# teenylasers/eggshell

Measured on AMD Instinct MI355X. Metric: constraint_solve_steps_per_sec, higher is better.
Workload: dtype f64

## Files before the change

### eggshell_amd/capi.py

```python
import ctypes as C
import ctypes as _ct
import os
import weakref

import numpy as np

_HERE = os.path.dirname(os.path.abspath(__file__))
LIB_PATH = os.path.join(_HERE, "libeggshell_amd.so")

OK, ERR_INVALID, ERR_NO_DEVICE, ERR_HIP, ERR_STALL, ERR_UNSUPPORTED, ERR_LCP_FAILED, ERR_INTERNAL = range(8)
JACOBI, GAUSS_SEIDEL, SOR = 0, 1, 2
F64, F32 = 0, 1
JOINT_BALL, CONTACT_BOX, JOINT_LOCK, JOINT_HINGE_AXIS = 0, 1, 2, 3
JOINT_SLIDER_AXIS = 5
SHAPE_BOX, SHAPE_SPHERE, SHAPE_CAPSULE = 0, 1, 2
MV_LOWER, MV_UPPER, MV_DIAG, MV_FULL = 1, 2, 4, 8
SCHED_QUAD, SCHED_ISO, SCHED_QUAD_PATCHES, SCHED_LANE_PATCHES, SCHED_ALL_GLOBAL, SCHED_STATIC, SCHED_LEAN = 1, 2, 4, 8, 16, 32, 64
SCHED_LINSYM = 128
SCHED_FUSED_ASSEMBLY = 256
SCHED_DEFERRED_SYSTEM = 512
SCHED_START = 1024
SCHED_FRICTION = 2048
SCHED_PAIR = 4096
SCHED_CHAIN = 8192
SCHED_SHARE = 16384
SCHED_FACE = 32768
SCHED_FACE_SPLIT = 65536
START_RHS, START_GIVEN, START_PREVIOUS = 0, 1, 2
STABILIZE_INIT, STABILIZE_POST = 0, 1

EXPORTS = [
    "egs_default_params", "egs_context_create", "egs_context_destroy", "egs_last_error",
    "egs_context_synchronize", "egs_timer_start", "egs_timer_stop", "egs_kernel_time",
    "egs_solve_blocks", "egs_problem_create", "egs_problem_create_batch", "egs_problem_destroy", "egs_problem_set_blocks",
    "egs_problem_solve", "egs_problem_get_lambda", "egs_problem_get_accumulators",
    "egs_problem_set_state", "egs_problem_set_mass", "egs_problem_set_constraints", "egs_problem_assemble",
    "egs_problem_step", "egs_problem_get_blocks", "egs_problem_get_velocity",
    "egs_problem_advance", "egs_problem_get_state",
    "egs_problem_get_stats", "egs_problem_get_schedule", "egs_problem_get_schedule_full", "egs_problem_get_schedule_forms", "egs_mixed_constraints_solve", "egs_debug_plan", "egs_debug_plan_slots",
    "egs_update_contacts", "egs_update_contacts_joints", "egs_world_create", "egs_world_destroy", "egs_world_set_bodies",
    "egs_world_set_joints", "egs_world_step", "egs_world_get_bodies", "egs_world_get_contacts",
    "egs_world_get_lambda", "egs_world_info", "egs_world_create_batch", "egs_world_batch_info",
    "egs_problem_matvec", "egs_problem_get_matvec", "egs_problem_get_wres", "egs_matvec_blocks",
    "egs_debug_matvec_plan", "egs_debug_choose_oversize_schedule", "egs_debug_plan_timetable", "egs_debug_plan_pairable", "egs_debug_plan_chained", "egs_debug_plan_share", "egs_debug_plan_faced", "egs_debug_plan_face_normals", "egs_debug_face_split", "egs_box_lcp_dantzig", "egs_box_lcp_murty",
    "egs_box_lcp_batch", "egs_box_lcp_schur", "egs_box_lcp_schur_batch", "egs_dense_condition", "egs_dense_iterate", "egs_dense_iterate_batch", "egs_debug_plan_patches", "egs_problem_debug_trace",
    "egs_mixed_constraints_solve_limits", "egs_mixed_constraints_solve_batch", "egs_problem_dense_system", "egs_problem_dense_condition", "egs_problem_step_dense",
    "egs_world_step_dense", "egs_world_dense_info", "egs_world_stabilize", "egs_world_stabilize_info",
    "egs_world_stabilize_direct", "egs_world_stabilize_rank", "egs_relax_blocks_direct",
    "egs_world_step_each", "egs_world_step_dense_each",
    "egs_problem_set_start", "egs_match_contacts", "egs_world_set_warm_start", "egs_world_get_start",
    "egs_problem_set_friction", "egs_world_set_friction",
    "egs_update_contacts_shapes", "egs_world_set_shapes",
    "egs_mixed_friction_solve_batch", "egs_problem_set_dense_friction", "egs_problem_dense_friction_info",
    "egs_world_set_dense_friction", "egs_world_dense_friction_info",
    "egs_problem_set_live_inertia", "egs_problem_get_mass", "egs_world_set_live_inertia", "egs_world_get_mass",
    "egs_problem_set_restitution", "egs_world_set_restitution",
    "egs_problem_set_motors", "egs_world_set_joints_kinds", "egs_world_set_joint_motors", "egs_world_get_blocks",
    "egs_problem_set_hinge_limits", "egs_world_set_joint_limits",
    "egs_problem_set_slider_limits", "egs_world_set_slider_limits",
# ... 225 lines not shown
        if self.h:
            for child in list(self._children):
                child.close()
            load().egs_context_destroy(self.h)
            self.h = C.c_void_p()

    def __del__(self):
        try:
            self.close()
        except Exception:
            pass

    def synchronize(self):
        self.check(load().egs_context_synchronize(self.h))

    def timer_start(self):
        self.check(load().egs_timer_start(self.h))

    def timer_stop(self):
        ms = C.c_float(0)
        self.check(load().egs_timer_stop(self.h, C.byref(ms)))
        return ms.value

    def kernel_time(self, reset=True):
        s = C.c_double(0); n = C.c_int64(0)
        self.check(load().egs_kernel_time(self.h, C.byref(s), C.byref(n), C.c_int(1 if reset else 0)))
        return s.value, n.value

    def solve_blocks(self, Minv, body0, body1, J0, J1, is_eq, lo, hi, rhs, prm, precision=F64):
        Minv, J0, J1, lo, hi, rhs = map(_f64, (Minv, J0, J1, lo, hi, rhs))
# ... 546 lines not shown
    return bool(out.value)


def debug_face_split(n_tiles, slots, depth, period, sweeps, force=None):
    h, s1 = (-1, 0) if force is None else force
    tiles, cut, n = C.c_int32(0), C.c_int32(0), C.c_int32(0)
    pieces = np.zeros((2 * max(int(n_tiles), 0) + 1, 4), dtype=np.int32)
    st = load().egs_debug_face_split(C.c_int32(n_tiles), C.c_int32(slots), C.c_int32(depth), C.c_int32(period),
                                     C.c_int32(sweeps), C.c_int32(h), C.c_int32(s1), C.byref(tiles), C.byref(cut),
                                     _p(pieces), C.byref(n))
    if st != OK:
        raise EgsError(st, "egs_debug_face_split failed")
    return tiles.value, cut.value, pieces[:n.value].copy()


def debug_plan_face_normals(n_bodies, body0, body1, data):
    body0, body1 = _i32(body0), _i32(body1)
    data = np.ascontiguousarray(data, dtype=np.float64).reshape(body0.shape[0], 7)
    out = C.c_int32(0)
    st = load().egs_debug_plan_face_normals(C.c_int32(n_bodies), C.c_int32(body0.shape[0]), _p(body0), _p(body1), _p(data),
                                            C.byref(out))
    if st != OK:
        raise EgsError(st, "egs_debug_plan_face_normals failed")
    return bool(out.value)


class World:

    def __init__(self, ctx, n_bodies, precision=F64, _handle=None):
        self.ctx, self.n = ctx, int(n_bodies)
# ... 231 lines not shown
```

### eggshell_amd/csrc/context.cpp

```cpp
#include "plan.h"
#include "runtime.h"

using namespace egs;

extern "C" {

void egs_default_params(egs_solve_params *p) {
  if (!p) return;
  p->method = EGS_GAUSS_SEIDEL;
  p->max_iters = 500;
  p->check_every = 1;
  p->reserved = 0;
  p->omega = 1.5;
  p->cfm = 0.0;
  p->tol = 1e-9;
}

egs_status egs_context_create(int device_index, egs_context **out) {
  if (!out) return EGS_ERR_INVALID;
  *out = nullptr;
  int count = 0;
  if (hipGetDeviceCount(&count) != hipSuccess || count <= 0) return EGS_ERR_NO_DEVICE;
  if (device_index < 0 || device_index >= count) return EGS_ERR_INVALID;
  egs_context *ctx = new (std::nothrow) egs_context;
// ... 30 lines not shown
  if (ctx->oneshot) { egs_problem_destroy(ctx->oneshot); ctx->oneshot = nullptr; }
  for (auto e : ctx->kev) if (e) (void)hipEventDestroy(e);
  if (ctx->t0) (void)hipEventDestroy(ctx->t0);
  if (ctx->t1) (void)hipEventDestroy(ctx->t1);
  if (ctx->stream) (void)hipStreamDestroy(ctx->stream);
  delete ctx;
}

const char *egs_last_error(const egs_context *ctx) { return ctx ? ctx->error.c_str() : "no context"; }

egs_status egs_context_synchronize(egs_context *ctx) {
  if (!ctx) return EGS_ERR_INVALID;
  return guarded(ctx, [&]() -> egs_status { HIPCHK(hipStreamSynchronize(ctx->stream)); return EGS_OK; });
}

egs_status egs_timer_start(egs_context *ctx) {
  if (!ctx) return EGS_ERR_INVALID;
  return guarded(ctx, [&]() -> egs_status { HIPCHK(hipEventRecord(ctx->t0, ctx->stream)); return EGS_OK; });
}

egs_status egs_timer_stop(egs_context *ctx, float *elapsed_ms) {
  if (!ctx || !elapsed_ms) return EGS_ERR_INVALID;
  return guarded(ctx, [&]() -> egs_status {
    HIPCHK(hipEventRecord(ctx->t1, ctx->stream));
    HIPCHK(hipEventSynchronize(ctx->t1));
    HIPCHK(hipEventElapsedTime(elapsed_ms, ctx->t0, ctx->t1));
    return EGS_OK;
  });
}

// ... 20 lines not shown
```

### eggshell_amd/csrc/kernels.h

```cpp
#pragma once
#include <hip/hip_runtime.h>

#include <cstdint>
#include <type_traits>

#include "plan.h"

namespace egs {

struct AssembleCore {
  int32_t n, m;
  const double *pos, *R, *v, *w;
  const double *Wf;
  const int32_t *kind, *body0, *body1;
  const double *data;
  double dt, erp;
  void *J0, *J1, *lo, *hi, *rhs;
  double *err;
  uint8_t *is_eq;
};
struct AssembleArgs : AssembleCore {
  const double *rest = nullptr;
  double vth = 0.0;
};
// ... 76 lines not shown
void launch_step_solve(const SolveArgs<REAL> &a, int method, int n_tiles, int block, int group, bool linsym, hipStream_t s);
void launch_step_solve_assemble(const SolveArgs<double> &a, int method, int n_tiles, bool store_system, hipStream_t s);
void launch_step_solve_pair(const SolveArgs<double> &a, int method, int n_tiles, bool store_system, bool chain, bool share,
                            hipStream_t s);
struct FacePiece;
struct FaceWork {
  const FacePiece *pieces;
  uint32_t *counter;
  uint32_t *flags;
  uint32_t ticket_base, epoch;
  int32_t n_pieces;
  int32_t n_workgroups;
  double *v6;
  int32_t *host_stall;
};
void launch_step_solve_face(const SolveArgs<double> &a, int n_tiles, int tiles_per_cu, const FaceWork &w, hipStream_t s);
template <typename REAL>
void launch_step_quad(const SolveArgs<REAL> &a, int method, int n_tiles, int tile_size, hipStream_t s);
template <typename REAL>
void launch_global_solve(const GlobalArgs<REAL> &a, int max_blocks, hipStream_t s);
template <typename REAL> int occupancy_global_solve();
template <typename REAL> int occupancy_patch_solve(size_t lds_bytes);
template <typename REAL> int occupancy_quad_patch_solve(size_t lds_bytes);
template <typename REAL> int occupancy_step_quad(int tile_size, size_t lds_bytes);
template <typename REAL>
void launch_global_wres(const GlobalArgs<REAL> &a, hipStream_t s);
template <typename REAL>
void launch_patch_solve(const SolveArgs<REAL> &a, int method, int n_tiles, uint32_t *tickets, hipStream_t s);
template <typename REAL>
void launch_cons_prepare(const SolveArgs<REAL> &a, hipStream_t s);
template <typename REAL>
// ... 70 lines not shown
```

### eggshell_amd/csrc/plan_debug.cpp

```cpp
#include <exception>

#include "../../include/eggshell_amd.h"
#include "matvec_plan.h"
#include "plan.h"
#include "policy.h"

using namespace egs;

namespace {

template <typename F>
egs_status plan_entry(int32_t n, int32_t m, const int32_t *body0, const int32_t *body1, F &&f) {
  if (n < 0 || m < 0 || (m > 0 && (!body0 || !body1))) return EGS_ERR_INVALID;
  try {
    return f();
  } catch (const std::exception &) {
    return EGS_ERR_INVALID;
  }
}

template <typename LANE, typename F>
void for_each_constraint_lane(const std::vector<LANE> &lanes, int n_tiles, int block, F &&f) {
  for (int t = 0; t < n_tiles; ++t)
    for (int l = 0; l < block; ++l) {
// ... 170 lines not shown
    if (s1) *s1 = f.s1;
    std::vector<FacePiece> list;
    face_piece_list(n_tiles, slots, f, sweeps, list);
    if (n_pieces) *n_pieces = (int32_t)list.size();
    if (pieces)
      for (size_t i = 0; i < list.size(); ++i) {
        pieces[4 * i] = list[i].tile; pieces[4 * i + 1] = list[i].resume;
        pieces[4 * i + 2] = list[i].sweeps; pieces[4 * i + 3] = list[i].kind;
      }
    return EGS_OK;
  } catch (const std::exception &) {
    return EGS_ERR_INVALID;
  }
}

}
```

### eggshell_amd/csrc/policy.h

```cpp
#pragma once

#include <algorithm>

#include "../../include/eggshell_amd.h"
#include "plan.h"

namespace egs {

inline int quad_tiles_per_cu_max(int precision) { return precision == EGS_F32 ? 8 : 5; }
constexpr int kBigTileMinConstraints = 196608;
inline bool timetable_pays(const Plan &pl, int sweeps) {
  const double grp = pl.runs ? 4.0 : 1.0;
  const double fixed = grp * ((double)pl.max_depth + (double)pl.max_period * sweeps);
  const double ticket = grp * (double)pl.max_depth + (double)pl.max_cnt * sweeps;
  return fixed <= 1.15 * ticket;
}

enum OversizeSchedule { kQuadPatches = 0, kLanePatches = 1, kAllGlobal = 2 };
inline OversizeSchedule choose_oversize_schedule(int n_patch_tiles, int quad_per_cu, int patch_per_cu, int cu_count,
                                                 bool patches_enabled, bool quad_patches_enabled) {
  if (n_patch_tiles <= 0 || !patches_enabled) return kAllGlobal;
  const long quad_cap = (long)std::min(quad_per_cu, 1) * cu_count, lane_cap = (long)std::min(patch_per_cu, 2) * cu_count;
  if (quad_patches_enabled && n_patch_tiles <= quad_cap) return kQuadPatches;
  if (n_patch_tiles <= lane_cap) return kLanePatches;
  return kAllGlobal;
}

constexpr int kFaceTilesPerCu = 4;

constexpr int kFaceSplitPrologueSteps = 260;
struct FaceSplit {
  int tiles = 0;
  int s1 = 0;
};
inline FaceSplit face_split_policy(long n_tiles, long slots, int depth, int P, int S) {
  FaceSplit f;
  if (slots <= 0 || n_tiles <= slots || S < 2 || P <= 0) return f;
  const long R = n_tiles % slots;
  if (R == 0 || 2 * R > slots) return f;
  const int s1 = S / 2;
  if ((long)P * (S - s1) <= (long)depth + kFaceSplitPrologueSteps) return f;
  f.tiles = (int)R;
  f.s1 = s1;
// ... 31 lines not shown
  for (long i = 0; i < total; ++i) {
    if (done_f < H && (done_w >= beside || done_f * total <= i * (long)H)) {
      out.push_back(FacePiece{whole + (int)done_f, 0, f.s1, kFaceFirst});
      ++done_f;
    } else {
      out.push_back(FacePiece{t++, 0, S, kFaceWhole});
      ++done_w;
    }
  }
  for (; t < whole; ++t) out.push_back(FacePiece{t, 0, S, kFaceWhole});
  for (int h = 0; h < H; ++h) out.push_back(FacePiece{whole + h, 1, S - f.s1, kFaceSecond});
}

inline bool face_persist_pays(long n_tiles, long slots) { return slots > 0 && n_tiles > slots; }

inline bool iso_schedule_pays(long m, int cu, int precision) {
  const long t = (m + 255) / 256;
  if (precision == EGS_F32) return t > 3L * cu;
  if (t < 2L * cu) return false;
  const long full3 = t / (3L * cu), rem3 = t % (3L * cu);
  const double iso = 0.50 * full3 + (rem3 == 0 ? 0.0 : rem3 <= cu ? 0.435 : rem3 <= 2L * cu ? 0.462 : 0.50);
  const double regular = 0.415 * ((t / 2 + cu - 1) / cu);
  return iso < regular;
}

}
```

### eggshell_amd/csrc/problem.h

```cpp
#pragma once

#include "kernels.h"
#include "matvec_plan.h"
#include "plan.h"
#include "policy.h"
#include "runtime.h"

namespace egs {

struct DevicePlan {
  DevBuf<LaneDesc> lanes;
  DevBuf<uint16_t> lane_level;
  DevBuf<int32_t> tile_period, tile_depth;
  DevBuf<int32_t> tile_nslots, tile_slot_off, slot_body;
  void stage(egs_context *ctx, const Plan &pl) {
    egs::stage(ctx, lanes, pl.lanes);
    egs::stage(ctx, lane_level, pl.lane_level);
    egs::stage(ctx, tile_period, pl.tile_period);
    egs::stage(ctx, tile_depth, pl.tile_depth);
    egs::stage(ctx, tile_nslots, pl.tile_nslots);
    egs::stage(ctx, tile_slot_off, pl.tile_slot_off);
    egs::stage(ctx, slot_body, pl.slot_body);
  }
};
// ... 10 lines not shown

}

struct egs_problem {
  egs_context *ctx = nullptr;
  int n = 0, m = 0, precision = EGS_F64;
  egs::Plan plan;
  bool tile_plan_ready = false;
  std::vector<int32_t> h_body0, h_body1;
  egs::DevicePlan tile;
  egs::Plan planq;
  bool use_quad = false;
  uint32_t last_sched = 0;
  static constexpr uint32_t kSchedRefinements = EGS_SCHED_CHAIN;
  static constexpr uint32_t kSchedFullOnly = EGS_SCHED_SHARE;
  static constexpr uint32_t kSchedFormsOnly = EGS_SCHED_FACE | EGS_SCHED_FACE_SPLIT;
  bool lin_neg = false;
  bool joint_pairs = false;
  bool contacts_only = false;
  int linsym_bodies = -1;
  static constexpr int kShareUndecided = -1, kShareDeviceData = -2;
  int share_normals = kShareDeviceData;
  bool face_normals = false;
  int oversize = 2;
  int global_max_blocks = 1;
  egs::DevicePlan quad;
  egs::DevBuf<unsigned char> wsB0, wsB1, wsD, wsInv;
  egs::DevBuf<egs::GlobalDesc> gcons;
  egs::DevBuf<uint32_t> gtickets;
  egs::DevBuf<unsigned long long> trace;
  int trace_sweeps = 0;
// ... 151 lines not shown
```

### eggshell_amd/csrc/solve.cpp

```cpp
#include <algorithm>
#include <cmath>
#include <cstdio>
#include <limits>

#include "policy.h"
#include "problem.h"
#include "stabilize.h"

namespace egs {
namespace {

struct SweepSchedule {
  bool quad = false;
  bool timetable = false;
  int iso = 0;
  int group = 1;
  bool linsym = false;
  bool assemble = false;
  bool defer = false;
  bool pair = false;
  bool chain = false;
  bool share = false;
  bool face = false;
  int face_tiles = kFaceTilesPerCu;
  FaceSplit split;
  long face_slots = 0;
  bool face_persistent = false;
  bool started = false;
  bool friction = false;
  int steady = 0;
  int oversize = -1;
  uint32_t flags() const {
    return (iso ? EGS_SCHED_ISO : 0) | (timetable ? EGS_SCHED_STATIC : 0) | (linsym ? EGS_SCHED_LINSYM : 0) |
           (assemble ? EGS_SCHED_FUSED_ASSEMBLY : 0) | (defer ? EGS_SCHED_DEFERRED_SYSTEM : 0) |
           (started ? EGS_SCHED_START : 0) | (friction ? EGS_SCHED_FRICTION : 0) | (pair ? EGS_SCHED_PAIR : 0) |
           (chain ? EGS_SCHED_CHAIN : 0) | (share ? EGS_SCHED_SHARE : 0) |
           (face ? EGS_SCHED_FACE : 0) | (split.tiles > 0 ? EGS_SCHED_FACE_SPLIT : 0);
  }
};

SweepSchedule choose_sweep(egs_problem *p, int method, int sweeps, bool hist, bool resume, bool offer_assembly) {
  SweepSchedule s;
  s.started = p->start_active;
  s.friction = p->friction;
  s.quad = p->use_quad && method != EGS_JACOBI;
  if (!s.quad) ensure_tile_plan(p);
  const Plan &pl = s.quad ? p->planq : p->plan;
  const char *se = std::getenv("EGS_STEP");
  s.timetable = method != EGS_JACOBI && pl.levels_ok && pl.n_tiles > 0 && (se ? std::atoi(se) != 0 : timetable_pays(pl, sweeps));
  if (s.quad) return s;
  const char *ye = std::getenv("EGS_STEP_STEADY");
  s.steady = s.timetable && !(ye && std::atoi(ye) == 0);
// ... 11 lines not shown
  s.linsym = !f32 && s.group == 1 && p->lin_neg && p->linsym_bodies == 1 && !(le && std::atoi(le) == 0);
  const char *fe = std::getenv("EGS_FUSED_ASSEMBLY");
  s.assemble = offer_assembly && s.linsym && p->contacts_only && !s.friction && !resume && !solve_takes_start(p) && pl.global.empty() && !(fe && std::atoi(fe) == 0);
  const char *de = std::getenv("EGS_STEP_DEFER_SYSTEM");
  s.defer = s.assemble && !(de && std::atoi(de) == 0);
  const char *pe = std::getenv("EGS_STEP_PAIR");
  s.pair = s.assemble && pl.pairable && !(pe && std::atoi(pe) == 0);
  const char *ce = std::getenv("EGS_STEP_CHAIN");
  s.chain = s.pair && pl.chained && s.steady && !(ce && std::atoi(ce) == 0);
  const char *he = std::getenv("EGS_STEP_SHARE");
  if (s.chain && p->share_normals == egs_problem::kShareUndecided) decide_share_normals(p);
  s.share = s.chain && p->share_normals == 1 && !(he && std::atoi(he) == 0);
  const char *ae = std::getenv("EGS_STEP_FACE"), *te = std::getenv("EGS_STEP_FACE_TILES");
  s.face = s.share && pl.faced && p->face_normals && method == EGS_GAUSS_SEIDEL && s.defer && !p->restitution &&
           !(ae && std::atoi(ae) == 0);
  if (te && (std::atoi(te) == 3 || std::atoi(te) == 4)) s.face_tiles = std::atoi(te);
  const char *xe = std::getenv("EGS_STEP_FACE_SPLIT"), *xf = std::getenv("EGS_STEP_FACE_SPLIT_FORCE");
  const char *ke = std::getenv("EGS_STEP_FACE_SLOTS");
  s.face_slots = ke && std::atol(ke) > 0 ? std::atol(ke) : (long)p->ctx->cu_count * s.face_tiles;
  if (s.face && !(xe && std::atoi(xe) == 0)) {
    long h = 0, s1 = 0;
    if (xf && std::sscanf(xf, "%ld,%ld", &h, &s1) == 2) s.split = face_split_forced(pl.n_tiles, h, s1, sweeps);
    else if (!xf) s.split = face_split_policy(pl.n_tiles, s.face_slots, pl.max_depth, pl.max_period, sweeps);
    const char *re = std::getenv("EGS_STEP_FACE_PERSIST");
    s.face_persistent = s.split.tiles > 0 || (face_persist_pays(pl.n_tiles, s.face_slots) && !(re && std::atoi(re) == 0));
  }
  return s;
}

template <typename ARGS, typename REAL>
void system_args(ARGS &a, const egs_problem *p, REAL cfm, bool hist) {
  a.m = p->m; a.n_bodies = p->n;
  a.Minv = real<REAL>(p->Minv_r);
// ... 69 lines not shown
  hipStream_t st = p->ctx->stream;
  if (!sc.assemble) {
    launch_step_solve<REAL>(a, method, n_tiles, p->plan.block, sc.group, sc.linsym, st);
    return;
  }
  if constexpr (sizeof(REAL) == 8) {
    a.assemble = *assemble;
    if (sc.face) {
      FaceWork w = sc.face_persistent ? face_work(p, n_tiles, sc.face_slots, sc.split, sweeps) : FaceWork{};
      w.host_stall = p->h_flag_dev;
      const char *ve = std::getenv("EGS_STEP_FACE_VELOCITY");
      if (p->step_velocity == egs_problem::kVelocityOffered && p->plan_covers_bodies && !(ve && std::atoi(ve) == 0)) {
        w.v6 = p->v6.p;
        p->step_velocity = egs_problem::kVelocityWritten;
      }
      launch_step_solve_face(a, n_tiles, sc.face_tiles, w, st);
    } else if (sc.pair) launch_step_solve_pair(a, method, n_tiles, !sc.defer, sc.chain, sc.share, st);
    else launch_step_solve_assemble(a, method, n_tiles, !sc.defer, st);
    p->sys_deferred = sc.defer;
    p->deferred_prev = false;
    p->deferred_dt = assemble->dt; p->deferred_erp = assemble->erp;
  }
}

template <typename REAL>
void launch_solve_t(egs_problem *p, int method, REAL cfm, REAL kscale, int sweeps, int resume, const AssembleArgs *assemble) {
  egs_context *ctx = p->ctx;
  const bool hist = p->hist_sweeps > 0;
  const SweepSchedule sc = choose_sweep(p, method, sweeps, hist, resume, assemble != nullptr);
  if (assemble && !sc.assemble)
    throw std::logic_error("fused assembly offered to a launch that does not take it");
// ... 495 lines not shown
```

### eggshell_amd/csrc/step_face.hip

```cpp
#include <algorithm>

#include "kernels.h"
#include "policy.h"
#include "step_device.h"
#include "step_pair_device.h"

namespace egs {

namespace {

#ifndef EGS_FACE_ANG_PRODUCTS
#define EGS_FACE_ANG_PRODUCTS 6
#endif
constexpr int kFaceLin = 9, kFaceAng = EGS_FACE_ANG_PRODUCTS;
constexpr int kFaceThreads = 128, kFaceLanes = 256;

struct FaceBodies {
  double pos0[3], pos1[3];
  double u0[6], u1[6];
  double wl0, wa0, wl1, wa1;
  bool has0, has1;
};
__device__ __forceinline__ void face_bodies(const SolveArgs<double> &A, int b0, int b1, FaceBodies &B) {
  const AssembleArgs &G = A.assemble;
  const size_t i0 = (size_t)max(b0, 0), i1 = (size_t)max(b1, 0);
  double vw0[6], vw1[6], wf0[6], wf1[6];
#pragma unroll
  for (int k = 0; k < 3; ++k) {
    B.pos0[k] = G.pos[i0 * 3 + k];
    B.pos1[k] = G.pos[i1 * 3 + k];
// ... 26 lines not shown
  double e[3];
  contact_blocks(d, B.pos0, B.pos1, has0, has1, c.J0, c.J1, e);
#pragma unroll
  for (int r = 0; r < 3; ++r) c.rhs[r] = assemble_rhs(A.assemble, c.J0, c.J1, e, B.u0, B.u1, r);
  c.wl0 = B.wl0; c.wa0 = B.wa0; c.wl1 = B.wl1; c.wa1 = B.wa1;
  load_cons<double, true, false, true, false, true>(A, 0, has0, has1, 0, 0, c);
#pragma unroll
  for (int r = 0; r < 3; ++r) {
    c.rhs[r] = active ? c.rhs[r] : 0.0;
    c.inv[r] = active ? c.inv[r] : 0.0;
    asm volatile("" : "+v"(c.rhs[r]), "+v"(c.inv[r]));
    x[r] = c.rhs[r];
  }
  asm volatile("" : "+v"(c.D[3]), "+v"(c.D[6]), "+v"(c.D[7]));
}
template <bool LIN>
__device__ __forceinline__ void face_sides(const Cons<double> &c, int side, PairLin<kFaceLin> &L, PairAng<kFaceAng> &GE,
                                           PairAng<kFaceAng> &GO) {
#pragma unroll
  for (int r = 0; r < 3; ++r) {
#pragma unroll
    for (int k = 0; k < 3; ++k) {
      const double ga = dpp_all<kQuadSwap>(side ? c.J0[6 * r + 3 + k] : c.J1[6 * r + 3 + k]);
      GE.J[3 * r + k] = side ? ga : c.J0[6 * r + 3 + k];
      GO.J[3 * r + k] = side ? c.J1[6 * r + 3 + k] : ga;
      if constexpr (LIN) {
        const double gl = dpp_all<kQuadSwap>(c.J1[6 * r + k]);
        L.J[3 * r + k] = side ? gl : c.J0[6 * r + k];
      }
    }
  }
  if constexpr (LIN) {
    const double gl = dpp_all<kQuadSwap>(c.wl1), ga = dpp_all<kQuadSwap>(c.wa1);
    L.wl = side ? gl : c.wl0;
    L.wa = side ? ga : c.wa0;
  }
}

template <bool PIECES>
__device__ __forceinline__ bool face_step(const SolveArgs<double> &A, const FaceWork &W, unsigned char *smem, const int tid) {
  constexpr int METHOD = 1;
  int tile = blockIdx.x, n_sweeps = A.sweeps, resume = 0, kind = kFaceWhole;
  if constexpr (PIECES) {
    unsigned *s_word = reinterpret_cast<unsigned *>(smem);
    if (tid == 0) *s_word = atomicAdd(W.counter, 1u) - W.ticket_base;
    __syncthreads();
    const unsigned ticket = (unsigned)__builtin_amdgcn_readfirstlane((int)*s_word);
    __syncthreads();
    if (ticket >= (unsigned)W.n_pieces) return false;
    const FacePiece pc = W.pieces[ticket];
    tile = __builtin_amdgcn_readfirstlane(pc.tile);
    resume = __builtin_amdgcn_readfirstlane(pc.resume);
    n_sweeps = __builtin_amdgcn_readfirstlane(pc.sweeps);
    kind = __builtin_amdgcn_readfirstlane(pc.kind);
  }
  const int side = tid & 1;
// ... 18 lines not shown

  const int own0 = side ? dm[1].cidx : dm[0].cidx, own1 = side ? dm[3].cidx : dm[2].cidx;
  double d0[7], d1[7];
#pragma unroll
  for (int k = 0; k < 7; ++k) {
    d0[k] = A.assemble.data[(size_t)max(own0, 0) * 7 + k];
    d1[k] = A.assemble.data[(size_t)max(own1, 0) * 7 + k];
  }
  const int body0 = slot_body[slot0], body1 = slot_body[slot1];
  __builtin_amdgcn_sched_barrier(0);
  FaceBodies B;
  B.has0 = slot0 != 0;
  B.has1 = slot1 != 0;
  face_bodies(A, body0, body1, B);

  PairLin<kFaceLin> L;
  PairAng<kFaceAng> GA, GB, GC, GD;
  Cons<double> c0 = {}, c1 = {};
  double x0[3], x1[3];
  face_assemble(A, d0, B, own0 >= 0, c0, x0);
  face_sides<true>(c0, side, L, GA, GB);
#pragma unroll
  for (int e = 0; e < 9; ++e) {
    s_acc[e * kFaceThreads + tid] = L.J[e];
    s_acc[(9 + e) * kFaceThreads + tid] = GA.J[e];
    s_acc[(18 + e) * kFaceThreads + tid] = GB.J[e];
  }
  asm volatile("" ::: "memory");
  __builtin_amdgcn_sched_barrier(0);
  face_assemble(A, d1, B, own1 >= 0, c1, x1);
  __builtin_amdgcn_sched_barrier(0);
  asm volatile("" ::: "memory");
#pragma unroll
  for (int e = 0; e < 9; ++e) {
    L.J[e] = s_acc[e * kFaceThreads + tid];
    GA.J[e] = s_acc[(9 + e) * kFaceThreads + tid];
    GB.J[e] = s_acc[(18 + e) * kFaceThreads + tid];
  }
  face_sides<false>(c1, side, L, GC, GD);
  __syncthreads();
  if (PIECES && resume) {
    unsigned *s_word = reinterpret_cast<unsigned *>(smem);
    if (tid == 0) {
      uint32_t spins = 0;
      unsigned ok = 1;
      while (__hip_atomic_load(W.flags + tile, __ATOMIC_ACQUIRE, __HIP_MEMORY_SCOPE_AGENT) != W.epoch) {
        if (++spins > A.spin_limit) { ok = 0; break; }
        __builtin_amdgcn_s_sleep(8);
      }
      *s_word = ok;
    }
    __syncthreads();
    const bool ok = __builtin_amdgcn_readfirstlane((int)*s_word) != 0;
    __builtin_amdgcn_fence(__ATOMIC_ACQUIRE, "agent");
    __syncthreads();
// ... 13 lines not shown
      const int body = slot_body[s];
#pragma unroll
      for (int k = 0; k < 6; ++k) s_acc[s * 6 + k] = body >= 0 ? A.acc[(size_t)body * 6 + k] : 0.0;
    }
  } else {
    for (int s = tid; s < nslots; s += kFaceThreads) {
#pragma unroll
      for (int k = 0; k < 6; ++k) s_acc[s * 6 + k] = 0.0;
    }
  }
  L.form();
  GA.form(L.wa);
  GB.form(L.wa);
  GC.form(L.wa);
  GD.form(L.wa);
  PairShared<kFaceLin, kFaceAng> SA{L, GA}, SB{L, GB}, SC{L, GC}, SD{L, GD};
  const int t_end = __builtin_amdgcn_readfirstlane(timetable_end<METHOD>(depth, P, n_sweeps, resume));
  __syncthreads();

  int sweep = resume, due = (nm > 0 && n_sweeps >= resume) ? levelA : 0x7fffffff;
  int t_s = 0, t_e = 0;
  const int Ps = __builtin_amdgcn_readfirstlane(P);
  if (A.steady && Ps > 0) {
    t_s = (__builtin_amdgcn_readfirstlane(depth) + 3) & ~3;
    t_e = min(Ps * (n_sweeps + 1 - resume), t_end);
    t_e -= (t_e - t_s) & 3;
    if (t_e <= t_s) t_s = t_e = 0;
  }
  int t = 0, stop = t_e > t_s ? t_s : t_end;
  double a[6];
  for (;;) {
    for (; t < stop; t += 4) {
      if (due == t) {
        pair_pass<METHOD, kQuadEven, true, true, false>(SA, ac, a, has, even, c0, x0, sweep, A.cfm);
        if (nm > 1) pair_pass<METHOD, kQuadOdd, true, false, false>(SB, ac, a, has, odd, c0, x0, sweep, A.cfm);
        if (nm > 2) pair_pass<METHOD, kQuadEven, true, false, false>(SC, ac, a, has, even, c1, x1, sweep, A.cfm);
        if (nm > 3) pair_pass<METHOD, kQuadOdd, true, false, false>(SD, ac, a, has, odd, c1, x1, sweep, A.cfm);
        if (has) store6(ac, a);
        due += P;
        if (++sweep > n_sweeps) due = 0x7fffffff;
      }
      asm volatile("s_waitcnt lgkmcnt(0)" ::: "memory");
      __builtin_amdgcn_s_barrier();
    }
    if (t >= t_end) break;
    {
      const int phF = nm > 0 ? levelA % Ps : -1;
      int tp = t % Ps;
      for (; t < t_e; t += 4) {
        if (phF == tp) {
          pair_pass<METHOD, kQuadEven, false, true, false>(SA, ac, a, has, even, c0, x0, 1, A.cfm);
          if (nm > 1) pair_pass<METHOD, kQuadOdd, false, false, false>(SB, ac, a, has, odd, c0, x0, 1, A.cfm);
          if (nm > 2) pair_pass<METHOD, kQuadEven, false, false, false>(SC, ac, a, has, even, c1, x1, 1, A.cfm);
          if (nm > 3) pair_pass<METHOD, kQuadOdd, false, false, false>(SD, ac, a, has, odd, c1, x1, 1, A.cfm);
          if (has) store6(ac, a);
        }
        asm volatile("s_waitcnt lgkmcnt(0)" ::: "memory");
        __builtin_amdgcn_s_barrier();
        tp = tp + 4 == Ps ? 0 : tp + 4;
      }
    }
    const int lv = A.lane_level[lane0];
    const int n = t_e > lv ? (t_e - lv + Ps - 1) / Ps : 0;
    sweep = n + resume;
    due = (nm == 0 || sweep > n_sweeps) ? 0x7fffffff : lv + P * n;
    stop = t_end;
  }

  const int cidx0 = A.lanes[lane0 + 32 * side].cidx, cidx1 = A.lanes[lane0 + 64 + 32 * side].cidx;
  if (nm > 0) pair_epilogue(A, SA, ac, even, cidx0, c0, x0);
  if (nm > 1) pair_epilogue(A, SB, ac, odd, cidx0, c0, x0);
  if (nm > 2) pair_epilogue(A, SC, ac, even, cidx1, c1, x1);
  if (nm > 3) pair_epilogue(A, SD, ac, odd, cidx1, c1, x1);
  for (int s = tid + 1; s < nslots; s += kFaceThreads) {
    const int body = slot_body[s];
    if (body < 0) continue;
    double acc[6];
#pragma unroll
    for (int k = 0; k < 6; ++k) A.acc[(size_t)body * 6 + k] = acc[k] = s_acc[s * 6 + k];
    if (W.v6 && kind != kFaceFirst) {
      const AssembleArgs &G = A.assemble;
#pragma unroll
      for (int k = 0; k < 6; ++k) {
        const double vel = k < 3 ? G.v[(size_t)body * 3 + k] : G.w[(size_t)body * 3 + k - 3];
        W.v6[(size_t)body * 6 + k] = vel + G.dt * (G.Wf[(size_t)body * 6 + k] + acc[k]);
      }
    }
  }
  if (PIECES && kind == kFaceFirst) {
    __builtin_amdgcn_fence(__ATOMIC_RELEASE, "agent");
    __syncthreads();
    if (tid == 0) __hip_atomic_store(W.flags + tile, W.epoch, __ATOMIC_RELEASE, __HIP_MEMORY_SCOPE_AGENT);
  }
  return true;
}

__global__ void __launch_bounds__(kFaceThreads, 2) step_solve_face_kernel(const SolveArgs<double> A, const FaceWork W) {
  extern __shared__ __attribute__((aligned(16))) unsigned char smem[];
  face_step<false>(A, W, smem, (int)threadIdx.x);
}
__global__ void __launch_bounds__(kFaceThreads, 2) step_solve_face_pieces_kernel(const SolveArgs<double> A, const FaceWork W) {
  extern __shared__ __attribute__((aligned(16))) unsigned char smem[];
  int tid = (int)threadIdx.x;
  for (;;) {
    SolveArgs<double> B = A;
    asm volatile("" : "+v"(tid), "+s"(B.assemble.dt), "+s"(B.assemble.erp), "+s"(B.cfm));
    if (!face_step<true>(B, W, smem, tid)) break;
    __syncthreads();
  }
}

}

void launch_step_solve_face(const SolveArgs<double> &a, int n_tiles, int tiles_per_cu, const FaceWork &w, hipStream_t s) {
  if (n_tiles <= 0) return;
  SolveArgs<double> b = a;
  b.n_tiles = n_tiles;
  size_t lds = std::max((size_t)b.max_slots * 6, (size_t)27 * kFaceThreads) * sizeof(double);
  constexpr size_t kQuarterLds = 160 * 1024 / 4;
  if (tiles_per_cu == 3) lds = std::max(lds, kQuarterLds + 1024);
  if (w.pieces) launch_lds(step_solve_face_pieces_kernel, dim3(w.n_workgroups), dim3(kFaceThreads), lds, s, b, w);
  else launch_lds(step_solve_face_kernel, dim3(n_tiles), dim3(kFaceThreads), lds, s, b, w);
}

}
```

### include/eggshell_amd.h

```cpp
#ifndef EGGSHELL_AMD_H
#define EGGSHELL_AMD_H

#include <stdint.h>

#ifdef __cplusplus
extern "C" {
#endif

typedef struct egs_context egs_context;
typedef struct egs_problem egs_problem;

typedef enum {
  EGS_OK = 0,
  EGS_ERR_INVALID = 1,
  EGS_ERR_NO_DEVICE = 2,
  EGS_ERR_HIP = 3,
  EGS_ERR_STALL = 4,
  EGS_ERR_UNSUPPORTED = 5,
  EGS_ERR_LCP_FAILED = 6,
  EGS_ERR_INTERNAL = 7
} egs_status;

typedef enum { EGS_JACOBI = 0, EGS_GAUSS_SEIDEL = 1, EGS_SOR = 2 } egs_method;
typedef enum { EGS_F64 = 0, EGS_F32 = 1 } egs_precision;
// ... 27 lines not shown
  EGS_SCHED_ISO = 2,
  EGS_SCHED_QUAD_PATCHES = 4,
  EGS_SCHED_LANE_PATCHES = 8,
  EGS_SCHED_ALL_GLOBAL = 16,
  EGS_SCHED_STATIC = 32,
  EGS_SCHED_LEAN = 64,
  EGS_SCHED_LINSYM = 128,
  EGS_SCHED_FUSED_ASSEMBLY = 256,
  EGS_SCHED_DEFERRED_SYSTEM = 512,
  EGS_SCHED_START = 1024,
  EGS_SCHED_FRICTION = 2048,
  EGS_SCHED_PAIR = 4096,
  EGS_SCHED_CHAIN = 8192,
  EGS_SCHED_SHARE = 16384,
  EGS_SCHED_FACE = 32768,
  EGS_SCHED_FACE_SPLIT = 65536
} egs_schedule_flags;

void egs_default_params(egs_solve_params *p);

egs_status egs_context_create(int device_index, egs_context **out);
void egs_context_destroy(egs_context *ctx);
const char *egs_last_error(const egs_context *ctx);
egs_status egs_context_synchronize(egs_context *ctx);
egs_status egs_timer_start(egs_context *ctx);
egs_status egs_timer_stop(egs_context *ctx, float *elapsed_ms);
egs_status egs_kernel_time(egs_context *ctx, double *sum_ms, int64_t *launches,
                           int reset);

egs_status egs_solve_blocks(egs_context *ctx, int32_t n_bodies,
                            const double *Minv, int32_t m,
                            const int32_t *body0, const int32_t *body1,
                            const double *J0, const double *J1,
                            const uint8_t *is_eq, const double *lo,
                            const double *hi, const double *rhs,
                            const egs_solve_params *params, int32_t precision,
                            double *x, egs_solve_stats *stats);

egs_status egs_problem_create(egs_context *ctx, int32_t n_bodies, int32_t m,
// ... 247 lines not shown
                                  int32_t *chained);

egs_status egs_debug_plan_share(int32_t n_bodies, int32_t m, const int32_t *body0, const int32_t *body1,
                                const double *data, int32_t *share);

egs_status egs_debug_plan_faced(int32_t n_bodies, int32_t m, const int32_t *body0, const int32_t *body1,
                                int32_t *faced);

egs_status egs_debug_plan_face_normals(int32_t n_bodies, int32_t m, const int32_t *body0, const int32_t *body1,
                                       const double *data, int32_t *face);

egs_status egs_debug_face_split(int32_t n_tiles, int32_t slots, int32_t depth, int32_t period, int32_t sweeps,
                                int32_t force_tiles, int32_t force_s1, int32_t *split_tiles, int32_t *s1,
                                int32_t *pieces, int32_t *n_pieces);

int32_t egs_debug_choose_oversize_schedule(int32_t n_patch_tiles, int32_t quad_per_cu,
                                           int32_t patch_per_cu, int32_t cu_count,
                                           int32_t patches_enabled, int32_t quad_patches_enabled);

egs_status egs_debug_matvec_plan(int32_t n_bodies, int32_t m, const int32_t *body0,
                                 const int32_t *body1, int32_t tile_size, int32_t *n_tiles,
                                 int32_t *n_islands, int32_t *n_shared_bodies,
                                 int32_t *n_boundary, int32_t *cons_tile, int32_t *cons_lane);

egs_status egs_cast_rays(egs_context *ctx, int32_t n_bodies, const double *pos, const double *R,
                         const double *side_lengths, const int32_t *shape ,
                         int32_t n_rays, const int32_t *ray_body ,
                         const double *origin, const double *dir, const double *tmax,
                         int32_t *hit_body, double *t, double *normal );
egs_status egs_world_set_rays(egs_world *w, int32_t n_rays, const int32_t *ray_ens ,
// ... 9 lines not shown
```

Before: 55770.

## Add lean FACE kernel variant with LDS-parked constraints for higher occupancy

Adds a lean form of the FACE step kernel that drops the angular product registers and parks per-constraint rhs, diagonal and inverse values in LDS, so it can run three workgroups per SIMD and six tiles per CU. A cost model (face_form_policy) picks lean or normal per problem by estimating launch time from piece count and block steps. The aim is higher occupancy and fewer persistent pieces on large problems. The price is extra LDS traffic on every pass and recomputed products, and lean is used only when the tile count exceeds the normal slot count and the model favours it.

```diff
diff --git a/eggshell_amd/capi.py b/eggshell_amd/capi.py
--- a/eggshell_amd/capi.py
+++ b/eggshell_amd/capi.py
@@ -26,12 +26,13 @@
 SCHED_SHARE = 16384
 SCHED_FACE = 32768
 SCHED_FACE_SPLIT = 65536
+SCHED_FACE_LEAN = 131072
 START_RHS, START_GIVEN, START_PREVIOUS = 0, 1, 2
 STABILIZE_INIT, STABILIZE_POST = 0, 1
 
 EXPORTS = [
     "egs_default_params", "egs_context_create", "egs_context_destroy", "egs_last_error",
-    "egs_context_synchronize", "egs_timer_start", "egs_timer_stop", "egs_kernel_time",
+    "egs_context_synchronize", "egs_context_cu_count", "egs_timer_start", "egs_timer_stop", "egs_kernel_time",
     "egs_solve_blocks", "egs_problem_create", "egs_problem_create_batch", "egs_problem_destroy", "egs_problem_set_blocks",
     "egs_problem_solve", "egs_problem_get_lambda", "egs_problem_get_accumulators",
     "egs_problem_set_state", "egs_problem_set_mass", "egs_problem_set_constraints", "egs_problem_assemble",
@@ -42,7 +43,7 @@
     "egs_world_set_joints", "egs_world_step", "egs_world_get_bodies", "egs_world_get_contacts",
     "egs_world_get_lambda", "egs_world_info", "egs_world_create_batch", "egs_world_batch_info",
     "egs_problem_matvec", "egs_problem_get_matvec", "egs_problem_get_wres", "egs_matvec_blocks",
-    "egs_debug_matvec_plan", "egs_debug_choose_oversize_schedule", "egs_debug_plan_timetable", "egs_debug_plan_pairable", "egs_debug_plan_chained", "egs_debug_plan_share", "egs_debug_plan_faced", "egs_debug_plan_face_normals", "egs_debug_face_split", "egs_box_lcp_dantzig", "egs_box_lcp_murty",
+    "egs_debug_matvec_plan", "egs_debug_choose_oversize_schedule", "egs_debug_plan_timetable", "egs_debug_plan_pairable", "egs_debug_plan_chained", "egs_debug_plan_share", "egs_debug_plan_faced", "egs_debug_plan_face_normals", "egs_debug_face_split", "egs_debug_face_form", "egs_box_lcp_dantzig", "egs_box_lcp_murty",
     "egs_box_lcp_batch", "egs_box_lcp_schur", "egs_box_lcp_schur_batch", "egs_dense_condition", "egs_dense_iterate", "egs_dense_iterate_batch", "egs_debug_plan_patches", "egs_problem_debug_trace",
     "egs_mixed_constraints_solve_limits", "egs_mixed_constraints_solve_batch", "egs_problem_dense_system", "egs_problem_dense_condition", "egs_problem_step_dense",
     "egs_world_step_dense", "egs_world_dense_info", "egs_world_stabilize", "egs_world_stabilize_info",
@@ -298,6 +299,11 @@
     def synchronize(self):
         self.check(load().egs_context_synchronize(self.h))
 
+    def cu_count(self):
+        n = C.c_int32(0)
+        self.check(load().egs_context_cu_count(self.h, C.byref(n)))
+        return n.value
+
     def timer_start(self):
         self.check(load().egs_timer_start(self.h))
 
@@ -874,6 +880,19 @@
     return tiles.value, cut.value, pieces[:n.value].copy()
 
 
+def debug_face_form(n_tiles, cus, depth, period, sweeps, max_slots=0):
+    lean, lds = C.c_int32(0), C.c_int64(0)
+    us, split = np.zeros(2, dtype=np.float64), np.zeros((2, 2), dtype=np.int32)
+    lib = load()
+    lib.egs_debug_face_form.argtypes = [C.c_int32] * 6 + [C.c_void_p] * 4
+    st = lib.egs_debug_face_form(n_tiles, cus, depth, period, sweeps, max_slots, C.addressof(lean), us.ctypes.data,
+                                 split.ctypes.data, C.addressof(lds))
+    if st != OK:
+        raise EgsError(st, "egs_debug_face_form failed")
+    return {"lean": bool(lean.value), "us": (float(us[0]), float(us[1])),
+            "split": (tuple(int(v) for v in split[0]), tuple(int(v) for v in split[1])), "lds_bytes": int(lds.value)}
+
+
 def debug_plan_face_normals(n_bodies, body0, body1, data):
     body0, body1 = _i32(body0), _i32(body1)
     data = np.ascontiguousarray(data, dtype=np.float64).reshape(body0.shape[0], 7)
diff --git a/eggshell_amd/csrc/context.cpp b/eggshell_amd/csrc/context.cpp
--- a/eggshell_amd/csrc/context.cpp
+++ b/eggshell_amd/csrc/context.cpp
@@ -68,6 +68,12 @@
   return guarded(ctx, [&]() -> egs_status { HIPCHK(hipStreamSynchronize(ctx->stream)); return EGS_OK; });
 }
 
+egs_status egs_context_cu_count(const egs_context *ctx, int32_t *cus) {
+  if (!ctx || !cus) return EGS_ERR_INVALID;
+  *cus = ctx->cu_count;
+  return EGS_OK;
+}
+
 egs_status egs_timer_start(egs_context *ctx) {
   if (!ctx) return EGS_ERR_INVALID;
   return guarded(ctx, [&]() -> egs_status { HIPCHK(hipEventRecord(ctx->t0, ctx->stream)); return EGS_OK; });
diff --git a/eggshell_amd/csrc/kernels.h b/eggshell_amd/csrc/kernels.h
--- a/eggshell_amd/csrc/kernels.h
+++ b/eggshell_amd/csrc/kernels.h
@@ -114,7 +114,8 @@
   double *v6;
   int32_t *host_stall;
 };
-void launch_step_solve_face(const SolveArgs<double> &a, int n_tiles, int tiles_per_cu, const FaceWork &w, hipStream_t s);
+void launch_step_solve_face(const SolveArgs<double> &a, int n_tiles, int tiles_per_cu, bool lean, const FaceWork &w,
+                            hipStream_t s);
 template <typename REAL>
 void launch_step_quad(const SolveArgs<REAL> &a, int method, int n_tiles, int tile_size, hipStream_t s);
 template <typename REAL>
diff --git a/eggshell_amd/csrc/plan_debug.cpp b/eggshell_amd/csrc/plan_debug.cpp
--- a/eggshell_amd/csrc/plan_debug.cpp
+++ b/eggshell_amd/csrc/plan_debug.cpp
@@ -208,4 +208,16 @@
   }
 }
 
-}
+egs_status egs_debug_face_form(int32_t n_tiles, int32_t cus, int32_t depth, int32_t period, int32_t sweeps,
+                               int32_t max_slots, int32_t *lean, double *us, int32_t *split, int64_t *lds_bytes) {
+  if (n_tiles < 0 || cus <= 0 || sweeps < 0) return EGS_ERR_INVALID;
+  const FaceForm f = face_form_policy(n_tiles, cus, depth, period, sweeps);
+  if (lean) *lean = f.lean ? 1 : 0;
+  if (us) { us[0] = f.us[0]; us[1] = f.us[1]; }
+  if (split)
+    for (int k = 0; k < 2; ++k) { split[2 * k] = f.split[k].tiles; split[2 * k + 1] = f.split[k].s1; }
+  if (lds_bytes) *lds_bytes = max_slots > 0 ? (int64_t)face_lds_bytes(max_slots, true, kFaceLeanTilesPerCu) : 0;
+  return EGS_OK;
+}
+
+}
diff --git a/eggshell_amd/csrc/policy.h b/eggshell_amd/csrc/policy.h
--- a/eggshell_amd/csrc/policy.h
+++ b/eggshell_amd/csrc/policy.h
@@ -27,6 +27,19 @@
 }
 
 constexpr int kFaceTilesPerCu = 4;
+
+constexpr int kFaceLeanTilesPerCu = 6;
+constexpr int kFaceTileThreads = 128;
+constexpr int kFaceStaged = 27, kFaceLeanStaged = 26, kFaceLeanParked = 18;
+constexpr size_t kCuLdsBytes = 160 * 1024, kFaceLeanLdsMax = 26 * 1024;
+inline size_t face_lds_bytes(int max_slots, bool lean, int tiles_per_cu) {
+  const size_t acc = (size_t)max_slots * 6, th = kFaceTileThreads;
+  size_t lds = (lean ? std::max(acc + kFaceLeanParked * th, kFaceLeanStaged * th) : std::max(acc, kFaceStaged * th)) * sizeof(double);
+  if (lean && lds > kFaceLeanLdsMax) return 0;
+  if (tiles_per_cu == 3) lds = std::max(lds, kCuLdsBytes / 4 + 1024);
+  else if (lean && tiles_per_cu == 4) lds = std::max(lds, kCuLdsBytes / 5 + 1024);
+  return lds;
+}
 
 constexpr int kFaceSplitPrologueSteps = 260;
 struct FaceSplit {
@@ -88,6 +101,36 @@
 
 inline bool face_persist_pays(long n_tiles, long slots) { return slots > 0 && n_tiles > slots; }
 
+constexpr double kFaceBlockUs = 0.93, kFacePieceUs = 28.0;
+constexpr double kFaceLeanBlockUs = 1.53, kFaceLeanPieceUs = 47.0;
+struct FaceForm {
+  bool lean = false;
+  double us[2] = {0.0, 0.0};
+  FaceSplit split[2];
+};
+inline double face_launch_us(long n_tiles, long slots, int depth, int P, int S, double block_us, double piece_us, FaceSplit &f) {
+  f = face_split_policy(n_tiles, slots, depth, P, S);
+  if (n_tiles <= 0 || slots <= 0) return 0.0;
+  const double tile = (double)depth + (double)P * S;
+  const long full = n_tiles / slots, rest = n_tiles % slots;
+  double steps = full * tile, pieces = (double)full;
+  if (f.tiles > 0) {
+    steps += (double)depth + (double)P * std::max(f.s1, S - f.s1) + kFaceSplitPrologueSteps;
+    pieces += 1;
+  } else if (rest > 0) {
+    steps += tile;
+    pieces += 1;
+  }
+  return pieces * piece_us + steps / 4 * block_us;
+}
+inline FaceForm face_form_policy(long n_tiles, int cus, int depth, int P, int S) {
+  FaceForm r;
+  r.us[0] = face_launch_us(n_tiles, (long)cus * kFaceTilesPerCu, depth, P, S, kFaceBlockUs, kFacePieceUs, r.split[0]);
+  r.us[1] = face_launch_us(n_tiles, (long)cus * kFaceLeanTilesPerCu, depth, P, S, kFaceLeanBlockUs, kFaceLeanPieceUs, r.split[1]);
+  r.lean = n_tiles > (long)cus * kFaceTilesPerCu && r.us[1] < r.us[0];
+  return r;
+}
+
 inline bool iso_schedule_pays(long m, int cu, int precision) {
   const long t = (m + 255) / 256;
   if (precision == EGS_F32) return t > 3L * cu;
diff --git a/eggshell_amd/csrc/problem.h b/eggshell_amd/csrc/problem.h
--- a/eggshell_amd/csrc/problem.h
+++ b/eggshell_amd/csrc/problem.h
@@ -48,7 +48,7 @@
   uint32_t last_sched = 0;
   static constexpr uint32_t kSchedRefinements = EGS_SCHED_CHAIN;
   static constexpr uint32_t kSchedFullOnly = EGS_SCHED_SHARE;
-  static constexpr uint32_t kSchedFormsOnly = EGS_SCHED_FACE | EGS_SCHED_FACE_SPLIT;
+  static constexpr uint32_t kSchedFormsOnly = EGS_SCHED_FACE | EGS_SCHED_FACE_SPLIT | EGS_SCHED_FACE_LEAN;
   bool lin_neg = false;
   bool joint_pairs = false;
   bool contacts_only = false;
diff --git a/eggshell_amd/csrc/solve.cpp b/eggshell_amd/csrc/solve.cpp
--- a/eggshell_amd/csrc/solve.cpp
+++ b/eggshell_amd/csrc/solve.cpp
@@ -22,6 +22,7 @@
   bool chain = false;
   bool share = false;
   bool face = false;
+  bool face_lean = false;
   int face_tiles = kFaceTilesPerCu;
   FaceSplit split;
   long face_slots = 0;
@@ -35,7 +36,8 @@
            (assemble ? EGS_SCHED_FUSED_ASSEMBLY : 0) | (defer ? EGS_SCHED_DEFERRED_SYSTEM : 0) |
            (started ? EGS_SCHED_START : 0) | (friction ? EGS_SCHED_FRICTION : 0) | (pair ? EGS_SCHED_PAIR : 0) |
            (chain ? EGS_SCHED_CHAIN : 0) | (share ? EGS_SCHED_SHARE : 0) |
-           (face ? EGS_SCHED_FACE : 0) | (split.tiles > 0 ? EGS_SCHED_FACE_SPLIT : 0);
+           (face ? EGS_SCHED_FACE : 0) | (split.tiles > 0 ? EGS_SCHED_FACE_SPLIT : 0) |
+           (face_lean ? EGS_SCHED_FACE_LEAN : 0);
   }
 };
 
@@ -77,9 +79,16 @@
   const char *ae = std::getenv("EGS_STEP_FACE"), *te = std::getenv("EGS_STEP_FACE_TILES");
   s.face = s.share && pl.faced && p->face_normals && method == EGS_GAUSS_SEIDEL && s.defer && !p->restitution &&
            !(ae && std::atoi(ae) == 0);
-  if (te && (std::atoi(te) == 3 || std::atoi(te) == 4)) s.face_tiles = std::atoi(te);
+  const char *ne = std::getenv("EGS_STEP_FACE_LEAN"), *ke = std::getenv("EGS_STEP_FACE_SLOTS");
+  const int tiles_env = te ? std::atoi(te) : 0, lean_env = ne ? std::atoi(ne) : -1;
+  if (s.face && lean_env != 0 && face_lds_bytes(pl.max_slots, true, kFaceLeanTilesPerCu) != 0) {
+    if (lean_env == 1 || tiles_env == kFaceLeanTilesPerCu) s.face_lean = true;
+    else if (lean_env < 0 && !te && !ke)
+      s.face_lean = face_form_policy(pl.n_tiles, p->ctx->cu_count, pl.max_depth, pl.max_period, sweeps).lean;
+  }
+  if (s.face_lean) s.face_tiles = kFaceLeanTilesPerCu;
+  if (tiles_env == 3 || tiles_env == 4) s.face_tiles = tiles_env;
   const char *xe = std::getenv("EGS_STEP_FACE_SPLIT"), *xf = std::getenv("EGS_STEP_FACE_SPLIT_FORCE");
-  const char *ke = std::getenv("EGS_STEP_FACE_SLOTS");
   s.face_slots = ke && std::atol(ke) > 0 ? std::atol(ke) : (long)p->ctx->cu_count * s.face_tiles;
   if (s.face && !(xe && std::atoi(xe) == 0)) {
     long h = 0, s1 = 0;
@@ -179,7 +188,7 @@
         w.v6 = p->v6.p;
         p->step_velocity = egs_problem::kVelocityWritten;
       }
-      launch_step_solve_face(a, n_tiles, sc.face_tiles, w, st);
+      launch_step_solve_face(a, n_tiles, sc.face_tiles, sc.face_lean, w, st);
     } else if (sc.pair) launch_step_solve_pair(a, method, n_tiles, !sc.defer, sc.chain, sc.share, st);
     else launch_step_solve_assemble(a, method, n_tiles, !sc.defer, st);
     p->sys_deferred = sc.defer;
diff --git a/eggshell_amd/csrc/step_face.hip b/eggshell_amd/csrc/step_face.hip
--- a/eggshell_amd/csrc/step_face.hip
+++ b/eggshell_amd/csrc/step_face.hip
@@ -1,4 +1,5 @@
 #include <algorithm>
+#include <stdexcept>
 
 #include "kernels.h"
 #include "policy.h"
@@ -14,6 +15,7 @@
 #endif
 constexpr int kFaceLin = 9, kFaceAng = EGS_FACE_ANG_PRODUCTS;
 constexpr int kFaceThreads = 128, kFaceLanes = 256;
+constexpr int kFaceLeanLin = 9, kFaceLeanLinPieces = 6;
 
 struct FaceBodies {
   double pos0[3], pos1[3];
@@ -70,9 +72,8 @@
   }
   asm volatile("" : "+v"(c.D[3]), "+v"(c.D[6]), "+v"(c.D[7]));
 }
-template <bool LIN>
-__device__ __forceinline__ void face_sides(const Cons<double> &c, int side, PairLin<kFaceLin> &L, PairAng<kFaceAng> &GE,
-                                           PairAng<kFaceAng> &GO) {
+template <bool LIN, int NL, int NA>
+__device__ __forceinline__ void face_sides(const Cons<double> &c, int side, PairLin<NL> &L, PairAng<NA> &GE, PairAng<NA> &GO) {
 #pragma unroll
   for (int r = 0; r < 3; ++r) {
 #pragma unroll
@@ -93,9 +94,34 @@
   }
 }
 
-template <bool PIECES>
+constexpr int kFaceOff[3] = {3, 6, 7};
+template <bool LEAN, int K>
+__device__ __forceinline__ void face_park(double *park, const Cons<double> &c) {
+  if constexpr (LEAN) {
+#pragma unroll
+    for (int r = 0; r < 3; ++r) {
+      park[(9 * K + r) * kFaceThreads] = c.rhs[r];
+      park[(9 * K + 3 + r) * kFaceThreads] = c.D[kFaceOff[r]];
+      park[(9 * K + 6 + r) * kFaceThreads] = c.inv[r];
+    }
+  }
+}
+template <bool LEAN, int K>
+__device__ __forceinline__ void face_unpark(const double *park, Cons<double> &c) {
+  if constexpr (LEAN) {
+#pragma unroll
+    for (int r = 0; r < 3; ++r) {
+      c.rhs[r] = park[(9 * K + r) * kFaceThreads];
+      c.D[kFaceOff[r]] = park[(9 * K + 3 + r) * kFaceThreads];
+      c.inv[r] = park[(9 * K + 6 + r) * kFaceThreads];
+    }
+  }
+}
+
+template <bool PIECES, bool LEAN>
 __device__ __forceinline__ bool face_step(const SolveArgs<double> &A, const FaceWork &W, unsigned char *smem, const int tid) {
   constexpr int METHOD = 1;
+  constexpr int NL = LEAN ? (PIECES ? kFaceLeanLinPieces : kFaceLeanLin) : kFaceLin, NA = LEAN ? 0 : kFaceAng;
   int tile = blockIdx.x, n_sweeps = A.sweeps, resume = 0, kind = kFaceWhole;
   if constexpr (PIECES) {
     unsigned *s_word = reinterpret_cast<unsigned *>(smem);
@@ -144,17 +170,19 @@
   B.has1 = slot1 != 0;
   face_bodies(A, body0, body1, B);
 
-  PairLin<kFaceLin> L;
-  PairAng<kFaceAng> GA, GB, GC, GD;
+  PairLin<NL> L;
+  PairAng<NA> GA, GB, GC, GD;
   Cons<double> c0 = {}, c1 = {};
   double x0[3], x1[3];
   face_assemble(A, d0, B, own0 >= 0, c0, x0);
   face_sides<true>(c0, side, L, GA, GB);
+  constexpr int SL = LEAN ? 8 : 9;
+  static_assert(SL + 18 == (LEAN ? kFaceLeanStaged : kFaceStaged), "policy.h sizes the staging");
 #pragma unroll
   for (int e = 0; e < 9; ++e) {
-    s_acc[e * kFaceThreads + tid] = L.J[e];
-    s_acc[(9 + e) * kFaceThreads + tid] = GA.J[e];
-    s_acc[(18 + e) * kFaceThreads + tid] = GB.J[e];
+    if (e < SL) s_acc[e * kFaceThreads + tid] = L.J[e];
+    s_acc[(SL + e) * kFaceThreads + tid] = GA.J[e];
+    s_acc[(SL + 9 + e) * kFaceThreads + tid] = GB.J[e];
   }
   asm volatile("" ::: "memory");
   __builtin_amdgcn_sched_barrier(0);
@@ -163,12 +191,19 @@
   asm volatile("" ::: "memory");
 #pragma unroll
   for (int e = 0; e < 9; ++e) {
-    L.J[e] = s_acc[e * kFaceThreads + tid];
-    GA.J[e] = s_acc[(9 + e) * kFaceThreads + tid];
-    GB.J[e] = s_acc[(18 + e) * kFaceThreads + tid];
+    if (e < SL) L.J[e] = s_acc[e * kFaceThreads + tid];
+    GA.J[e] = s_acc[(SL + e) * kFaceThreads + tid];
+    GB.J[e] = s_acc[(SL + 9 + e) * kFaceThreads + tid];
   }
   face_sides<false>(c1, side, L, GC, GD);
   __syncthreads();
+  static_assert(kFaceLeanParked == 18, "policy.h sizes the parked values");
+  double *s_park = nullptr;
+  if constexpr (LEAN) {
+    s_park = s_acc + (size_t)A.max_slots * 6 + tid;
+    face_park<LEAN, 0>(s_park, c0);
+    face_park<LEAN, 1>(s_park, c1);
+  }
   if (PIECES && resume) {
     unsigned *s_word = reinterpret_cast<unsigned *>(smem);
     if (tid == 0) {
@@ -212,7 +247,7 @@
   GB.form(L.wa);
   GC.form(L.wa);
   GD.form(L.wa);
-  PairShared<kFaceLin, kFaceAng> SA{L, GA}, SB{L, GB}, SC{L, GC}, SD{L, GD};
+  PairShared<NL, NA> SA{L, GA}, SB{L, GB}, SC{L, GC}, SD{L, GD};
   const int t_end = __builtin_amdgcn_readfirstlane(timetable_end<METHOD>(depth, P, n_sweeps, resume));
   __syncthreads();
 
@@ -230,8 +265,10 @@
   for (;;) {
     for (; t < stop; t += 4) {
       if (due == t) {
+        face_unpark<LEAN, 0>(s_park, c0);
         pair_pass<METHOD, kQuadEven, true, true, false>(SA, ac, a, has, even, c0, x0, sweep, A.cfm);
         if (nm > 1) pair_pass<METHOD, kQuadOdd, true, false, false>(SB, ac, a, has, odd, c0, x0, sweep, A.cfm);
+        face_unpark<LEAN, 1>(s_park, c1);
         if (nm > 2) pair_pass<METHOD, kQuadEven, true, false, false>(SC, ac, a, has, even, c1, x1, sweep, A.cfm);
         if (nm > 3) pair_pass<METHOD, kQuadOdd, true, false, false>(SD, ac, a, has, odd, c1, x1, sweep, A.cfm);
         if (has) store6(ac, a);
@@ -247,8 +284,10 @@
       int tp = t % Ps;
       for (; t < t_e; t += 4) {
         if (phF == tp) {
+          face_unpark<LEAN, 0>(s_park, c0);
           pair_pass<METHOD, kQuadEven, false, true, false>(SA, ac, a, has, even, c0, x0, 1, A.cfm);
           if (nm > 1) pair_pass<METHOD, kQuadOdd, false, false, false>(SB, ac, a, has, odd, c0, x0, 1, A.cfm);
+          face_unpark<LEAN, 1>(s_park, c1);
           if (nm > 2) pair_pass<METHOD, kQuadEven, false, false, false>(SC, ac, a, has, even, c1, x1, 1, A.cfm);
           if (nm > 3) pair_pass<METHOD, kQuadOdd, false, false, false>(SD, ac, a, has, odd, c1, x1, 1, A.cfm);
           if (has) store6(ac, a);
@@ -266,6 +305,8 @@
   }
 
   const int cidx0 = A.lanes[lane0 + 32 * side].cidx, cidx1 = A.lanes[lane0 + 64 + 32 * side].cidx;
+  face_unpark<LEAN, 0>(s_park, c0);
+  face_unpark<LEAN, 1>(s_park, c1);
   if (nm > 0) pair_epilogue(A, SA, ac, even, cidx0, c0, x0);
   if (nm > 1) pair_epilogue(A, SB, ac, odd, cidx0, c0, x0);
   if (nm > 2) pair_epilogue(A, SC, ac, even, cidx1, c1, x1);
@@ -295,7 +336,7 @@
 
 __global__ void __launch_bounds__(kFaceThreads, 2) step_solve_face_kernel(const SolveArgs<double> A, const FaceWork W) {
   extern __shared__ __attribute__((aligned(16))) unsigned char smem[];
-  face_step<false>(A, W, smem, (int)threadIdx.x);
+  face_step<false, false>(A, W, smem, (int)threadIdx.x);
 }
 __global__ void __launch_bounds__(kFaceThreads, 2) step_solve_face_pieces_kernel(const SolveArgs<double> A, const FaceWork W) {
   extern __shared__ __attribute__((aligned(16))) unsigned char smem[];
@@ -303,22 +344,38 @@
   for (;;) {
     SolveArgs<double> B = A;
     asm volatile("" : "+v"(tid), "+s"(B.assemble.dt), "+s"(B.assemble.erp), "+s"(B.cfm));
-    if (!face_step<true>(B, W, smem, tid)) break;
-    __syncthreads();
-  }
-}
-
-}
-
-void launch_step_solve_face(const SolveArgs<double> &a, int n_tiles, int tiles_per_cu, const FaceWork &w, hipStream_t s) {
+    if (!face_step<true, false>(B, W, smem, tid)) break;
+    __syncthreads();
+  }
+}
+__global__ void __launch_bounds__(kFaceThreads, 3) step_solve_face_lean_kernel(const SolveArgs<double> A, const FaceWork W) {
+  extern __shared__ __attribute__((aligned(16))) unsigned char smem[];
+  face_step<false, true>(A, W, smem, (int)threadIdx.x);
+}
+__global__ void __launch_bounds__(kFaceThreads, 3) step_solve_face_lean_pieces_kernel(const SolveArgs<double> A, const FaceWork W) {
+  extern __shared__ __attribute__((aligned(16))) unsigned char smem[];
+  int tid = (int)threadIdx.x;
+  for (;;) {
+    SolveArgs<double> B = A;
+    asm volatile("" : "+v"(tid), "+s"(B.assemble.dt), "+s"(B.assemble.erp), "+s"(B.cfm));
+    if (!face_step<true, true>(B, W, smem, tid)) break;
+    __syncthreads();
+  }
+}
+
+}
+
+void launch_step_solve_face(const SolveArgs<double> &a, int n_tiles, int tiles_per_cu, bool lean, const FaceWork &w,
+                            hipStream_t s) {
   if (n_tiles <= 0) return;
   SolveArgs<double> b = a;
   b.n_tiles = n_tiles;
-  size_t lds = std::max((size_t)b.max_slots * 6, (size_t)27 * kFaceThreads) * sizeof(double);
-  constexpr size_t kQuarterLds = 160 * 1024 / 4;
-  if (tiles_per_cu == 3) lds = std::max(lds, kQuarterLds + 1024);
-  if (w.pieces) launch_lds(step_solve_face_pieces_kernel, dim3(w.n_workgroups), dim3(kFaceThreads), lds, s, b, w);
-  else launch_lds(step_solve_face_kernel, dim3(n_tiles), dim3(kFaceThreads), lds, s, b, w);
-}
-
-}
+  static_assert(kFaceThreads == kFaceTileThreads, "policy.h sizes the LDS request for this many threads");
+  const size_t lds = face_lds_bytes(b.max_slots, lean, tiles_per_cu);
+  if (lds == 0) throw std::logic_error("a lean FACE launch asked for where a tile's LDS request does not fit");
+  auto *kernel = w.pieces ? (lean ? step_solve_face_lean_pieces_kernel : step_solve_face_pieces_kernel)
+                          : (lean ? step_solve_face_lean_kernel : step_solve_face_kernel);
+  launch_lds(kernel, w.pieces ? dim3(w.n_workgroups) : dim3(n_tiles), dim3(kFaceThreads), lds, s, b, w);
+}
+
+}
diff --git a/include/eggshell_amd.h b/include/eggshell_amd.h
--- a/include/eggshell_amd.h
+++ b/include/eggshell_amd.h
@@ -65,7 +65,8 @@
   EGS_SCHED_CHAIN = 8192,
   EGS_SCHED_SHARE = 16384,
   EGS_SCHED_FACE = 32768,
-  EGS_SCHED_FACE_SPLIT = 65536
+  EGS_SCHED_FACE_SPLIT = 65536,
+  EGS_SCHED_FACE_LEAN = 131072
 } egs_schedule_flags;
 
 void egs_default_params(egs_solve_params *p);
@@ -74,6 +75,7 @@
 void egs_context_destroy(egs_context *ctx);
 const char *egs_last_error(const egs_context *ctx);
 egs_status egs_context_synchronize(egs_context *ctx);
+egs_status egs_context_cu_count(const egs_context *ctx, int32_t *cus);
 egs_status egs_timer_start(egs_context *ctx);
 egs_status egs_timer_stop(egs_context *ctx, float *elapsed_ms);
 egs_status egs_kernel_time(egs_context *ctx, double *sum_ms, int64_t *launches,
@@ -351,6 +353,9 @@
                                 int32_t force_tiles, int32_t force_s1, int32_t *split_tiles, int32_t *s1,
                                 int32_t *pieces, int32_t *n_pieces);
 
+egs_status egs_debug_face_form(int32_t n_tiles, int32_t cus, int32_t depth, int32_t period, int32_t sweeps,
+                               int32_t max_slots, int32_t *lean, double *us, int32_t *split, int64_t *lds_bytes);
+
 int32_t egs_debug_choose_oversize_schedule(int32_t n_patch_tiles, int32_t quad_per_cu,
                                            int32_t patch_per_cu, int32_t cu_count,
                                            int32_t patches_enabled, int32_t quad_patches_enabled);
```

After: 62650, median of 6. 1.12x the previous value.
